# magicat777/Audio-Analyzer-OMEGA

Measured on NVIDIA B200. Metric: stream-seconds of 48 kHz stereo analysed/sec (multi-res FFT+LUFS+TP), higher is better.
Workload: dtype f32 (FFT, combine, K-weighting in a float32 delta-form state, sample peaks of the true-peak meter; its four transforms per frame pair in f16x2; tensor-core GEMM on (hi, lo) half operands with fp32 accumulators for the few-bin resolutions) + f64 (meter statistics)

## Files before the change

audio-analyzer-omega_b200/csrc/omega4_cuda.cu:

```cuda
#include "../../include/omega4_cuda.h"

#include <cuda_runtime.h>
#include <math.h>
#include <stdio.h>
#include <stdlib.h>
#include <string.h>

#include <algorithm>
#include <map>
#include <mutex>
#include <set>
#include <string>
#include <vector>

#include "bars_kernel.cuh"
#include "blockdft_kernel.cuh"
#include "blockdft_tc_kernel.cuh"
#include "fft_core.cuh"
#include "kweight_kernel.cuh"
#include "kweight32_kernel.cuh"
#include "misc_kernels.cuh"
#include "multires_kernel.cuh"
#include "stats_kernel.cuh"
#include "truepeak_kernel.cuh"
#include "truepeak16_kernel.cuh"
#include "waterfall_kernel.cuh"

using namespace o4;

static thread_local std::string g_err;

static int fail(int code, const std::string& msg) {
    g_err = msg;
    return code;
}
#define CK(expr)                                                                                   \
    do {                                                                                           \
        cudaError_t e__ = (expr);                                                                  \
        if (e__ != cudaSuccess) {                                                                  \
            char b__[512];                                                                         \
            snprintf(b__, sizeof b__, "%s failed: %s (%s:%d)", #expr, cudaGetErrorString(e__),     \
                     __FILE__, __LINE__);                                                          \
            return fail(OMEGA4_ERR_CUDA, b__);                                                     \
        }                                                                                          \
    } while (0)

extern "C" const char* omega4_last_error(void) { return g_err.c_str(); }
extern "C" int omega4_abi_version(void) { return OMEGA4_ABI_VERSION; }
extern "C" int omega4_device_count(void) {
    int n = 0;
    if (cudaGetDeviceCount(&n) != cudaSuccess) { cudaGetLastError(); return 0; }
    return n;
}

static int ilog2(int n) { int l = 0; while ((1 << l) < n) ++l; return l; }
static bool is_pow2(int n) { return n > 0 && (n & (n - 1)) == 0; }

struct Twiddles { float2* twM = nullptr; float2* twN = nullptr; float2* tw4W = nullptr; };
static std::mutex g_tw_mu;
static std::map<std::pair<int, int>, Twiddles> g_tw;

static int get_twiddles(int device, int log2m, Twiddles* out) {
    std::lock_guard<std::mutex> lk(g_tw_mu);
    auto key = std::make_pair(device, log2m);
    auto it = g_tw.find(key);
    if (it != g_tw.end()) { *out = it->second; return OMEGA4_OK; }
    const int M = 1 << log2m, N = 2 * M;
    const double two_pi = 6.283185307179586476925287;
    std::vector<float2> a(M), b(M / 2 + 1), c(3 * M + 1);
    for (int e = 0; e < M; ++e) a[e] = make_float2((float)cos(two_pi * e / M), (float)-sin(two_pi * e / M));
    for (int k = 0; k <= M / 2; ++k) b[k] = make_float2((float)cos(two_pi * k / N), (float)-sin(two_pi * k / N));
    for (int j = 0; j <= 3 * M; ++j) c[j] = make_float2((float)cos(two_pi * j / (4.0 * N)), (float)sin(two_pi * j / (4.0 * N)));
    Twiddles t;
    CK(cudaMalloc(&t.twM, a.size() * sizeof(float2)));
    CK(cudaMalloc(&t.twN, b.size() * sizeof(float2)));
    CK(cudaMalloc(&t.tw4W, c.size() * sizeof(float2)));
    CK(cudaMemcpy(t.twM, a.data(), a.size() * sizeof(float2), cudaMemcpyHostToDevice));
    CK(cudaMemcpy(t.twN, b.data(), b.size() * sizeof(float2), cudaMemcpyHostToDevice));
    CK(cudaMemcpy(t.tw4W, c.data(), c.size() * sizeof(float2), cudaMemcpyHostToDevice));
    g_tw[key] = t;
    *out = t;
    return OMEGA4_OK;
}

template <int L>
static int launch_multires_t(const MultiresArgs& a, cudaStream_t s) {
    using S = FftShape<L>;
    const int fpc = a.rounds * S::CONC;
    const long long tiles = (a.n_frames + fpc - 1) / fpc;
    const long long grid = tiles * a.n_ch;
    if (grid <= 0) return OMEGA4_OK;
    if (grid > 2147483647LL) return fail(OMEGA4_ERR_INVALID, "multires grid too large");
    if constexpr (L <= 12) {
        const size_t smem = multires_local_smem_bytes<L>(a.need_cnt, a.n_tb);
        CK(cudaFuncSetAttribute(multires_local_kernel<L>, cudaFuncAttributeMaxDynamicSharedMemorySize, (int)smem));
        multires_local_kernel<L><<<(unsigned)grid, 256, smem, s>>>(a);
    } else {
        const size_t smem = multires_smem_bytes<L>(a.need_cnt);
        CK(cudaFuncSetAttribute(multires_kernel<L>, cudaFuncAttributeMaxDynamicSharedMemorySize, (int)smem));
        multires_kernel<L><<<(unsigned)grid, S::NT, smem, s>>>(a);
    }
    CK(cudaGetLastError());
    return OMEGA4_OK;
}

static int launch_multires(int log2m, const MultiresArgs& a, cudaStream_t s) {
    switch (log2m) {
        case 8: return launch_multires_t<8>(a, s);
        case 9: return launch_multires_t<9>(a, s);
        case 10: return launch_multires_t<10>(a, s);
        case 11: return launch_multires_t<11>(a, s);
        case 12: return launch_multires_t<12>(a, s);
        case 13: return launch_multires_t<13>(a, s);
        case 14: return launch_multires_t<14>(a, s);
    }
    return fail(OMEGA4_ERR_UNSUPPORTED, "fft size must be a power of two in 512 .. 32768");
}

static int default_rounds(int n_frames, int conc) {
    int r = 16;
    while (r > 1 && (long long)r * conc > n_frames) r >>= 1;
    return r;
}

static void fill_truepeak_steps(TruePeakArgs* t) {
    const double two_pi = 6.283185307179586476925287;
    for (int p = 1; p <= 3; ++p) {
        for (int j = 0; j < 16; ++j) {
            const int jj = j < 8 ? j : j - 16;
            t->step[p - 1][j] = make_float2((float)cos(two_pi * p * jj / 64.0), (float)sin(two_pi * p * jj / 64.0));
        }
        t->nyq[p - 1] = (float)cos(two_pi * p / 8.0);
    }
}

static int launch_truepeak(const TruePeakArgs& a, cudaStream_t s) {
    constexpr int L = 11;
    using S = FftShape<L>;
    const size_t smem = truepeak_smem_bytes<L>();
    CK(cudaFuncSetAttribute(truepeak_kernel<L>, cudaFuncAttributeMaxDynamicSharedMemorySize, (int)smem));
    const int ppc = a.rounds * S::CONC;
    const int n_pairs = (a.n_frames + 1) / 2;
    const long long grid = (long long)((n_pairs + ppc - 1) / ppc) * a.n_ch;
    if (grid <= 0) return OMEGA4_OK;
    if (grid > 2147483647LL) return fail(OMEGA4_ERR_INVALID, "truepeak grid too large");
    truepeak_kernel<L><<<(unsigned)grid, S::NT, smem, s>>>(a);
    CK(cudaGetLastError());
    return OMEGA4_OK;
}

static int launch_truepeak16(const TruePeakArgs& a, cudaStream_t s) {
    constexpr int L = 11;
    using S = FftShape<L>;
    const size_t smem = truepeak16_smem_bytes<L>();
    CK(cudaFuncSetAttribute(truepeak16_kernel<L>, cudaFuncAttributeMaxDynamicSharedMemorySize, (int)smem));
    const int ppc = a.rounds * S::CONC;
    const int n_pairs = (a.n_frames + 1) / 2;
    const long long grid = (long long)((n_pairs + ppc - 1) / ppc) * a.n_ch;
    if (grid <= 0) return OMEGA4_OK;
    if (grid > 2147483647LL) return fail(OMEGA4_ERR_INVALID, "truepeak grid too large");
    truepeak16_kernel<L><<<(unsigned)grid, S::NT, smem, s>>>(a);
    CK(cudaGetLastError());
    return OMEGA4_OK;
}

template <bool F64, bool WT>
static int launch_kweight_t(const KweightArgs& a, cudaStream_t s) {
    const size_t smem = kweight_smem_bytes();
    CK(cudaFuncSetAttribute(kweight_kernel<F64, WT>, cudaFuncAttributeMaxDynamicSharedMemorySize, (int)smem));
    const int fpc = a.frames_per_warp * KW_WARPS;
    const long long grid = (long long)((a.n_frames + fpc - 1) / fpc) * a.n_ch;
    if (grid <= 0) return OMEGA4_OK;
    if (grid > 2147483647LL) return fail(OMEGA4_ERR_INVALID, "kweight grid too large");
    kweight_kernel<F64, WT><<<(unsigned)grid, KW_WARPS * 32, smem, s>>>(a);
    CK(cudaGetLastError());
    return OMEGA4_OK;
}

static int launch_kweight(const KweightArgs& a, cudaStream_t s) {
    if (a.x_is_f64) return a.weighted_out ? launch_kweight_t<true, true>(a, s) : launch_kweight_t<true, false>(a, s);
    return a.weighted_out ? launch_kweight_t<false, true>(a, s) : launch_kweight_t<false, false>(a, s);
}

static int launch_kweight32(const Kweight32Args& a, cudaStream_t s) {
    const size_t smem = kweight32_smem_bytes();
    CK(cudaFuncSetAttribute(kweight32_kernel, cudaFuncAttributeMaxDynamicSharedMemorySize, (int)smem));
    const int fpc = a.frames_per_warp * KW32_WARPS;
    const long long grid = (long long)((a.n_frames + fpc - 1) / fpc) * a.n_ch;
    if (grid <= 0) return OMEGA4_OK;
    if (grid > 2147483647LL) return fail(OMEGA4_ERR_INVALID, "kweight grid too large");
    kweight32_kernel<<<(unsigned)grid, KW32_WARPS * 32, smem, s>>>(a);
    CK(cudaGetLastError());
    return OMEGA4_OK;
}

static int launch_stats(const StatsArgs& a, cudaStream_t s) {
    if (a.n_ch <= 0) return OMEGA4_OK;
    if (!a.fresh && a.n_frames == 1 && a.first_frame == 0 && !getenv("OMEGA4_STATS_WALK")) {
        stats_push1_kernel<<<a.n_ch, ST_P1_THREADS, 0, s>>>(a);
    } else if (a.fresh) {
        const size_t smem = stats_smem_bytes<false>();
        CK(cudaFuncSetAttribute(stats_kernel<false>, cudaFuncAttributeMaxDynamicSharedMemorySize, (int)smem));
        stats_kernel<false><<<a.n_ch, ST_THREADS, smem, s>>>(a);
    } else {
        const size_t smem = stats_smem_bytes<true>();
        CK(cudaFuncSetAttribute(stats_kernel<true>, cudaFuncAttributeMaxDynamicSharedMemorySize, (int)smem));
        stats_kernel<true><<<a.n_ch, ST_THREADS, smem, s>>>(a);
    }
    CK(cudaGetLastError());
    return OMEGA4_OK;
}

static int launch_s16_convert(const int16_t* in, long long stream_stride, int il, int n_streams, long long n_frames,
                              float* out, long long out_stride, cudaStream_t s) {
    if (n_streams <= 0 || n_frames <= 0) return OMEGA4_OK;
    if (n_streams > 65535) return fail(OMEGA4_ERR_INVALID, "too many streams for one int16 conversion launch (max 65535)");
    const long long per_stream = n_frames * il;
    dim3 grid((unsigned)((per_stream + 1023) / 1024), (unsigned)n_streams);
    s16_deinterleave_kernel<<<grid, 256, 0, s>>>(in, stream_stride, il, n_frames, out, out_stride);
    CK(cudaGetLastError());
    return OMEGA4_OK;
}

static void mat2_mul(const double* a, const double* b, double* c) {
    double r[4] = {a[0] * b[0] + a[1] * b[2], a[0] * b[1] + a[1] * b[3],
                   a[2] * b[0] + a[3] * b[2], a[2] * b[1] + a[3] * b[3]};
    memcpy(c, r, sizeof r);
}

static void build_biquad(const double* b, const double* a, int order, KwBiquad* q) {
    memset(q, 0, sizeof *q);
    const double a0 = a[0];
    q->b0 = b[0] / a0; q->b1 = b[1] / a0; q->b2 = order >= 2 ? b[2] / a0 : 0.0;
    q->a1 = a[1] / a0; q->a2 = order >= 2 ? a[2] / a0 : 0.0;
    q->pad = 3 * (order + 1);
    if (order >= 2) {
        double zi0, zi1;
        const double m00 = 1.0 + q->a1, m01 = -1.0, m10 = q->a2, m11 = 1.0;
        const double r0 = q->b1 - q->a1 * q->b0, r1 = q->b2 - q->a2 * q->b0;
        const double det = m00 * m11 - m01 * m10;
        zi0 = (r0 * m11 - m01 * r1) / det;
        zi1 = (m00 * r1 - m10 * r0) / det;
        q->yi0 = -zi1 / q->a2;
        q->yi1 = (-zi0 + q->a1 * zi1 / q->a2) / q->a2;
// ... 81 lines not shown
        return OMEGA4_OK;
    }
    void release() { if (p) cudaFree(p); p = nullptr; cap = 0; }
};

struct omega4_bars {
    int device = 0, T = 0, n_valid = 0, p_lo = 0, normalize_max = 0;
    float p_frac = 0.f, scale = 0.8f;
    int* bands = nullptr; float* gain = nullptr; float* sf = nullptr; float* sfc = nullptr;
    DevBuf h_spec, h_out, h_peak, h_state, state_in;
};

static int bars_launch(omega4_bars* b, cudaStream_t s, const float* spec, int n_ch, int n_hops, float* state, int fresh,
                       float* band_values, float* peak_values, DevBuf* state_copy) {
    BarsArgs a;
    memset(&a, 0, sizeof a);
    a.T = b->T; a.n_ch = n_ch; a.n_hops = n_hops; a.n_valid = b->n_valid; a.bands = b->bands; a.gain = b->gain;
    a.sf = b->sf; a.sfc = b->sfc; a.p_lo = b->p_lo; a.p_frac = b->p_frac; a.scale = b->scale;
    a.normalize_max = b->normalize_max; a.fresh = (fresh || !state) ? 1 : 0;
    a.spec = spec; a.bars_out = band_values; a.peaks_out = peak_values; a.state = state;
    const size_t st_bytes = (size_t)n_ch * (1 + b->n_valid) * sizeof(float);
    const size_t smem = bars_smem_bytes(b->T, b->n_valid);
    if (smem > 200 * 1024) return fail(OMEGA4_ERR_UNSUPPORTED, "spectrum too long for the bars kernel");
    if (b->T > 32 * BARS_MAXV) return fail(OMEGA4_ERR_UNSUPPORTED, "spectrum too long for the bars kernel (max 1024 bins)");
    if (b->T <= 512) CK(cudaFuncSetAttribute(bars_kernel<16>, cudaFuncAttributeMaxDynamicSharedMemorySize, (int)smem));
    else CK(cudaFuncSetAttribute(bars_kernel<32>, cudaFuncAttributeMaxDynamicSharedMemorySize, (int)smem));
    a.seg = n_ch >= 1024 ? 4 * BARS_SEG : BARS_SEG;
    const long long grid = (long long)n_ch * ((n_hops + a.seg - 1) / a.seg);
    if (grid > 2147483647LL) return fail(OMEGA4_ERR_INVALID, "bars grid too large");
    if (a.state && !a.fresh && n_hops > a.seg) {
        int rc = state_copy->ensure(st_bytes); if (rc) return rc;
        CK(cudaMemcpyAsync(state_copy->p, a.state, st_bytes, cudaMemcpyDeviceToDevice, s));
        a.state_in = (const float*)state_copy->p;
    }
    if (b->T <= 512) bars_kernel<16><<<(unsigned)grid, BARS_WARPS * 32, smem, s>>>(a);
    else bars_kernel<32><<<(unsigned)grid, BARS_WARPS * 32, smem, s>>>(a);
    CK(cudaGetLastError());
    return OMEGA4_OK;
}

struct BarsReq {
    omega4_bars* b = nullptr;
    float* band_values = nullptr; float* peak_values = nullptr; float* state = nullptr;
    int fresh = 1;
};

struct KernelTime { char name[32]; cudaEvent_t e0, e1; };

struct SideCtx {
    cudaStream_t side = nullptr;
    cudaEvent_t ev_fork = nullptr, ev_tp = nullptr, ev_join = nullptr;
    int ensure() {
        if (side) return OMEGA4_OK;
        CK(cudaStreamCreateWithFlags(&side, cudaStreamNonBlocking));
        CK(cudaEventCreateWithFlags(&ev_fork, cudaEventDisableTiming));
        CK(cudaEventCreateWithFlags(&ev_tp, cudaEventDisableTiming));
        CK(cudaEventCreateWithFlags(&ev_join, cudaEventDisableTiming));
        return OMEGA4_OK;
    }
    void release() {
        if (side) cudaStreamDestroy(side);
        if (ev_fork) cudaEventDestroy(ev_fork);
        if (ev_tp) cudaEventDestroy(ev_tp);
        if (ev_join) cudaEventDestroy(ev_join);
        side = nullptr; ev_fork = ev_tp = ev_join = nullptr;
    }
};

struct omega4_plan {
    int device = 0;
    int sample_rate = 48000, hop = 512, n_res = 0, T = 0, W = OMEGA4_METER_WINDOW;
    double gate = -70.0;
    ResInfo res[OMEGA4_MAX_RES];
    bool disjoint = true;
    int* csr_ptr = nullptr; int* csr_res = nullptr; int* csr_lo = nullptr; float* csr_frac = nullptr;
    double* hann64 = nullptr;
    float* hann32 = nullptr;
    KwBiquad kw_default[2];
    KwBiquad kw[4];
    int kw_nsec = 2, kw_blend = 1, kw_gate = 1;
    double kw_gain = 1.0;
    Twiddles tw_meter;
    float2* tp_rot = nullptr;
    unsigned* tp_rot_h = nullptr;
    SparseSet set_cc;
    SparseSet set_tc;
    bool tensor_default = true;
    DevBuf scratch_lufs, scratch_tp, scratch_mag[OMEGA4_MAX_RES], scratch_q, scratch_f32, scratch_comb, scratch_bstate, scratch_inv;
    DevBuf h_in, h_comb, h_meters, h_state, h_mag[OMEGA4_MAX_RES], h_f64a, h_f64b, h_f64c;
    struct Slot {
        cudaStream_t s = nullptr;
        DevBuf in, in16, comb, met, lufs, tp, state, q, mag[OMEGA4_MAX_RES];
        DevBuf bars, peaks, bstate, bstate_copy;
        SideCtx sc;
    };
#ifndef OMEGA4_HOST_SLOTS
#define OMEGA4_HOST_SLOTS 4
#endif
    static constexpr int N_SLOTS = OMEGA4_HOST_SLOTS;
    Slot slots[N_SLOTS];
    size_t host_chunk_bytes = (size_t)1024 << 20;
    SideCtx sc;
    long long launches = 0;
    std::vector<KernelTime> times;
    size_t n_times = 0;
};

static void set_weighting_k(omega4_plan* p) {
    p->kw[0] = p->kw_default[0]; p->kw[1] = p->kw_default[1];
    p->kw_nsec = 2; p->kw_blend = 1; p->kw_gate = 1; p->kw_gain = 1.0;
}

static double max_pole_radius(const KwBiquad& q) {
    if (q.a2 == 0.0) return fabs(q.a1);
    const double disc = q.a1 * q.a1 - 4.0 * q.a2;
    if (disc < 0.0) return sqrt(q.a2);
    return fmax(fabs(-q.a1 + sqrt(disc)), fabs(-q.a1 - sqrt(disc))) * 0.5;
}

static void to_float(const KwBiquad& s, KwBiquadF* d) {
    d->b0 = (float)s.b0; d->b1 = (float)s.b1; d->b2 = (float)s.b2; d->a1 = (float)s.a1; d->a2 = (float)s.a2;
    d->yi0 = (float)s.yi0; d->yi1 = (float)s.yi1; d->pad = s.pad; d->_align = 0;
    for (int j = 0; j < 5; ++j) for (int e = 0; e < 4; ++e) d->phi[j][e] = (float)s.phi[j][e];
    for (int e = 0; e < 4; ++e) {
        d->cinv_f[e] = (float)s.cinv_f[e]; d->cinv_b[e] = (float)s.cinv_b[e];
        d->c16[e] = (float)s.c16[e]; d->c17[e] = (float)s.c17[e];
    }
    for (int i = 0; i < KW_SUBMAX; ++i) { d->g[i][0] = (float)s.g[i][0]; d->g[i][1] = (float)s.g[i][1]; }
}

static bool is_highpass_biquad(const KwBiquad& q) {
    return q.pad == 9 && q.a2 != 0.0 && fabs(q.b1 + 2.0 * q.b0) <= 1e-12 * fabs(q.b0) && fabs(q.b2 - q.b0) <= 1e-12 * fabs(q.b0);
}

static void build_kw32(const KwBiquad& q, Kw32Sec* o) {
    const double alpha = 1.0 + q.a1 + q.a2, beta = 1.0 - q.a2;
    const double bb = -q.b0 * beta, gamma = alpha / bb;
    o->b0 = (float)q.b0; o->a2 = (float)q.a2; o->gamma = (float)gamma; o->bb = (float)bb;
    const double M[4] = {1.0 - alpha, bb * q.a2, -gamma, q.a2};
    double P[4] = {M[0], M[1], M[2], M[3]};
    for (int i = 0; i < KW_L; ++i) {
        if (i < KW_SUBMAX) { o->g[i][0] = (float)P[0]; o->g[i][1] = (float)P[1]; }
        if (i + 1 == 16) for (int e = 0; e < 4; ++e) o->c16[e] = (float)P[e];
        if (i + 1 == 17) for (int e = 0; e < 4; ++e) o->c17[e] = (float)P[e];
        if (i + 1 < KW_L) mat2_mul(M, P, P);
    }
    for (int k = 0; k < 16; ++k) {
        o->ga0[k] = make_float2(o->g[k + 1][0], o->g[k][0]);
        o->ga1[k] = make_float2(o->g[k + 1][1], o->g[k][1]);
    }
    double Q[4] = {P[0], P[1], P[2], P[3]};
    for (int j = 0; j < 5; ++j) {
        for (int e = 0; e < 4; ++e) o->phi[j][e] = (float)Q[e];
        mat2_mul(Q, Q, Q);
    }
}

static bool use_kweight32(const omega4_plan* p) {
    return p->W == KW_W && p->kw_nsec == 2 && p->kw_blend && p->kw_gain == 1.0 && is_highpass_biquad(p->kw[0]) &&
           is_highpass_biquad(p->kw[1]) && !getenv("OMEGA4_KW_F64");
}

static void fill_weighting(const omega4_plan* p, KweightArgs* k) {
    k->n_sec = p->kw_nsec; k->blend = p->kw_blend; k->rms_gate = p->kw_gate; k->gain = p->kw_gain;
    for (int i = 0; i < p->kw_nsec; ++i) { k->f[i] = p->kw[i]; to_float(p->kw[i], &k->ff[i]); }
    int from = p->kw_nsec;
    while (from > 1 && max_pole_radius(p->kw[from - 1]) < 0.95) --from;
// ... 237 lines not shown
    size_t woff = 0, boff = 0, toff = 0;
    std::vector<std::vector<int>> idx(d->n_res), lo(d->n_res);
    std::vector<std::vector<float>> fr(d->n_res);
    for (int r = 0; r < d->n_res; ++r) {
        ResInfo& ri = p->res[r];
        const int n = d->fft_sizes[r];
        if (!is_pow2(n) || n < 512 || n > 32768) return fail(OMEGA4_ERR_UNSUPPORTED, "fft size must be a power of two in 512 .. 32768");
        ri.n = n; ri.log2m = ilog2(n) - 1; ri.bins = n / 2 + 1; ri.weight = d->res_weight[r];
        if (ri.weight <= 0.f) return fail(OMEGA4_ERR_INVALID, "resolution weight must be positive");
        int rc = upload((void**)&ri.window, d->windows + woff, (size_t)n * sizeof(float));
        if (rc) return rc;
        if (d->bin_weights) { rc = upload((void**)&ri.binw, d->bin_weights + boff, (size_t)ri.bins * sizeof(float)); if (rc) return rc; }
        woff += n; boff += ri.bins;
        const int cnt = d->tb_count[r];
        if (cnt < 0) return fail(OMEGA4_ERR_INVALID, "negative tb_count");
        for (int j = 0; j < cnt; ++j) {
            const int ti = d->tb_idx[toff + j], l = d->tb_lo[toff + j];
            if (ti < 0 || ti >= d->target_bins || l < 0 || l + 1 >= ri.bins)
                return fail(OMEGA4_ERR_INVALID, "combine table entry out of range");
            idx[r].push_back(ti); lo[r].push_back(l); fr[r].push_back(d->tb_frac[toff + j]);
            owners[ti]++;
        }
        toff += cnt;
        rc = get_twiddles(p->device, ri.log2m, &ri.tw);
        if (rc) return rc;
    }
    p->disjoint = true;
    for (int t = 0; t < d->target_bins; ++t) if (owners[t] > 1) p->disjoint = false;
    {
        std::vector<int> ptr(d->target_bins + 1, 0), cres, clo;
        std::vector<float> cfr;
        for (int t = 0; t < d->target_bins; ++t) {
            for (int r = 0; r < d->n_res; ++r)
                for (size_t j = 0; j < idx[r].size(); ++j)
                    if (idx[r][j] == t) { cres.push_back(r); clo.push_back(lo[r][j]); cfr.push_back(fr[r][j]); }
            ptr[t + 1] = (int)cres.size();
        }
        int rc = upload((void**)&p->csr_ptr, ptr.data(), ptr.size() * sizeof(int)); if (rc) return rc;
        rc = upload((void**)&p->csr_res, cres.data(), cres.size() * sizeof(int)); if (rc) return rc;
        rc = upload((void**)&p->csr_lo, clo.data(), clo.size() * sizeof(int)); if (rc) return rc;
        rc = upload((void**)&p->csr_frac, cfr.data(), cfr.size() * sizeof(float)); if (rc) return rc;
    }
    for (int r = 0; r < d->n_res; ++r) {
        ResInfo& ri = p->res[r];
        int mn = 1 << 30, mx = -1;
        for (int l : lo[r]) { if (l < mn) mn = l; if (l > mx) mx = l; }
        if (mx >= 0) { ri.need_lo = mn; ri.need_cnt = mx + 2 - mn; } else { ri.need_lo = 0; ri.need_cnt = 0; }
        if (r == 0)
            for (int t = 0; t < d->target_bins; ++t)
                if (owners[t] == 0) { idx[0].push_back(t); lo[0].push_back(-1); fr[0].push_back(0.f); }
        ri.n_tb = (int)idx[r].size();
        int rc = upload((void**)&ri.tb_idx, idx[r].data(), idx[r].size() * sizeof(int)); if (rc) return rc;
        rc = upload((void**)&ri.tb_lo, lo[r].data(), lo[r].size() * sizeof(int)); if (rc) return rc;
        rc = upload((void**)&ri.tb_frac, fr[r].data(), fr[r].size() * sizeof(float)); if (rc) return rc;
    }
    if (p->disjoint) {
        int rc = build_sparse_set(p, d, idx, lo, false, &p->set_cc); if (rc) return rc;
        rc = build_sparse_set(p, d, idx, lo, true, &p->set_tc); if (rc) return rc;
    }
    int rc = upload((void**)&p->hann64, d->meter_hann, (size_t)p->W * sizeof(double)); if (rc) return rc;
    std::vector<float> h32(p->W);
    for (int i = 0; i < p->W; ++i) h32[i] = (float)d->meter_hann[i];
    rc = upload((void**)&p->hann32, h32.data(), h32.size() * sizeof(float)); if (rc) return rc;
    build_biquad(d->kw_coeffs + 0, d->kw_coeffs + 3, 2, &p->kw_default[0]);
    build_biquad(d->kw_coeffs + 6, d->kw_coeffs + 9, 2, &p->kw_default[1]);
    set_weighting_k(p);
    rc = get_twiddles(p->device, ilog2(p->W), &p->tw_meter); if (rc) return rc;
    {
        const int W = p->W;
        std::vector<float2> rot((size_t)3 * W);
        const double two_pi = 6.283185307179586476925287;
        for (int ph = 1; ph <= 3; ++ph)
            for (int k = 0; k < W; ++k) {
                float2 v;
                if (k == W / 2) v = make_float2((float)cos(two_pi * ph / 8.0), 0.f);
                else {
                    const double f = (k < W / 2) ? (double)k : (double)k - W;
                    const double ang = two_pi * f * ph / (4.0 * W);
                    v = make_float2((float)cos(ang), (float)sin(ang));
                }
                rot[(size_t)(ph - 1) * W + k] = v;
            }
        rc = upload((void**)&p->tp_rot, rot.data(), rot.size() * sizeof(float2)); if (rc) return rc;
        std::vector<unsigned> roth(rot.size());
        for (size_t i = 0; i < rot.size(); ++i) {
            const __half2 h = __floats2half2_rn(rot[i].x, rot[i].y);
            memcpy(&roth[i], &h, sizeof(unsigned));
        }
        rc = upload((void**)&p->tp_rot_h, roth.data(), roth.size() * sizeof(unsigned)); if (rc) return rc;
    }
    return OMEGA4_OK;
}

extern "C" omega4_plan* omega4_plan_create(const omega4_plan_desc* desc, int device) {
    if (!desc) { fail(OMEGA4_ERR_INVALID, "desc is NULL"); return nullptr; }
    int ndev = 0;
    if (cudaGetDeviceCount(&ndev) != cudaSuccess || ndev == 0) {
        cudaGetLastError();
        fail(OMEGA4_ERR_NO_DEVICE, "no CUDA device visible: libomega4_cuda has no CPU fallback");
        return nullptr;
    }
    if (device < 0 || device >= ndev) { fail(OMEGA4_ERR_INVALID, "bad device index"); return nullptr; }
    if (cudaSetDevice(device) != cudaSuccess) { fail(OMEGA4_ERR_CUDA, "cudaSetDevice failed"); return nullptr; }
    omega4_plan* p = new omega4_plan();
    p->device = device;
    if (const char* e = getenv("OMEGA4_TENSOR")) p->tensor_default = atoi(e) != 0;
    if (const char* e = getenv("OMEGA4_HOST_CHUNK_MB")) {
        long mb = atol(e);
        if (mb >= 16 && mb <= 16384) p->host_chunk_bytes = (size_t)mb << 20;
    }
    if (plan_build(p, desc) != OMEGA4_OK) { std::string keep = g_err; omega4_plan_destroy(p); g_err = keep; return nullptr; }
    return p;
}

static void stream_ctx_release(omega4_plan* p);

extern "C" void omega4_plan_destroy(omega4_plan* p) {
    if (!p) return;
    cudaSetDevice(p->device);
    stream_ctx_release(p);
    for (int r = 0; r < OMEGA4_MAX_RES; ++r) {
        ResInfo& ri = p->res[r];
        cudaFree(ri.window); cudaFree(ri.binw); cudaFree(ri.tb_idx); cudaFree(ri.tb_lo); cudaFree(ri.tb_frac);
        p->scratch_mag[r].release(); p->h_mag[r].release();
    }
    cudaFree(p->csr_ptr); cudaFree(p->csr_res); cudaFree(p->csr_lo); cudaFree(p->csr_frac);
    cudaFree(p->hann64); cudaFree(p->hann32); cudaFree(p->tp_rot); cudaFree(p->tp_rot_h);
    p->scratch_lufs.release(); p->scratch_tp.release(); p->scratch_q.release(); p->scratch_f32.release(); p->scratch_inv.release();
    p->scratch_comb.release(); p->scratch_bstate.release();
    p->set_cc.release(); p->set_tc.release();
    p->h_in.release(); p->h_comb.release(); p->h_meters.release(); p->h_state.release();
    p->h_f64a.release(); p->h_f64b.release(); p->h_f64c.release();
    for (auto& sl : p->slots) {
        sl.in.release(); sl.comb.release(); sl.met.release(); sl.lufs.release(); sl.tp.release(); sl.state.release();
        sl.q.release(); sl.in16.release(); sl.sc.release();
        sl.bars.release(); sl.peaks.release(); sl.bstate.release(); sl.bstate_copy.release();
        for (auto& m : sl.mag) m.release();
        if (sl.s) cudaStreamDestroy(sl.s);
    }
    for (auto& t : p->times) { cudaEventDestroy(t.e0); cudaEventDestroy(t.e1); }
    p->sc.release();
    cudaGetLastError();
    delete p;
}

extern "C" long long omega4_plan_launches(const omega4_plan* p) { return p ? p->launches : 0; }

extern "C" int omega4_plan_set_weighting(omega4_plan* p, const omega4_weighting* w) {
    if (!p) return fail(OMEGA4_ERR_INVALID, "plan is NULL");
    if (!w) { set_weighting_k(p); return OMEGA4_OK; }
    if (w->n_sections < 0 || w->n_sections > 4) return fail(OMEGA4_ERR_INVALID, "0..4 weighting sections");
    if (w->blend && w->n_sections != 2) return fail(OMEGA4_ERR_INVALID, "the K blend needs exactly two sections");
    KwBiquad tmp[4];
    for (int i = 0; i < w->n_sections; ++i) {
        const int order = w->order[i];
        if (order != 1 && order != 2) return fail(OMEGA4_ERR_UNSUPPORTED, "weighting sections must be first or second order");
        if (w->a[i][0] == 0.0 || w->a[i][1] == 0.0 || (order == 2 && w->a[i][2] == 0.0))
            return fail(OMEGA4_ERR_UNSUPPORTED, "weighting sections need non-zero denominator coefficients");
        build_biquad(w->b[i], w->a[i], order, &tmp[i]);
    }
    for (int i = 0; i < w->n_sections; ++i) p->kw[i] = tmp[i];
    p->kw_nsec = w->n_sections; p->kw_blend = w->blend ? 1 : 0; p->kw_gate = w->rms_gate ? 1 : 0;
    p->kw_gain = w->blend ? 1.0 : w->gain;
    return OMEGA4_OK;
}

struct Bracket {
    omega4_plan* p; cudaStream_t s; bool on; KernelTime* kt = nullptr;
    Bracket(omega4_plan* p_, cudaStream_t s_, bool on_, const char* name) : p(p_), s(s_), on(on_) {
        p->launches++;
        if (!on) return;
        if (p->n_times == p->times.size()) {
            KernelTime t; memset(&t, 0, sizeof t);
            cudaEventCreate(&t.e0); cudaEventCreate(&t.e1);
            p->times.push_back(t);
        }
        kt = &p->times[p->n_times++];
        snprintf(kt->name, sizeof kt->name, "%s", name);
        cudaEventRecord(kt->e0, s);
    }
    ~Bracket() { if (on && kt) cudaEventRecord(kt->e1, s); }
};

extern "C" int omega4_plan_kernel_times(omega4_plan* p, char* names, float* ms, int max_n) {
    if (!p) return fail(OMEGA4_ERR_INVALID, "plan is NULL");
    int n = 0;
    for (size_t i = 0; i < p->n_times && n < max_n; ++i, ++n) {
        float t = 0.f;
        if (cudaEventElapsedTime(&t, p->times[i].e0, p->times[i].e1) != cudaSuccess) { cudaGetLastError(); t = -1.f; }
        if (names) { memcpy(names + 32 * n, p->times[i].name, 32); }
        if (ms) ms[n] = t;
    }
    return n;
}

template <int BN>
static int launch_blockdft_gemm_t(const BlockDftGemmArgs& a, cudaStream_t s) {
    const size_t smem = blockdft_gemm_smem_bytes<BN>();
    CK(cudaFuncSetAttribute(blockdft_gemm_kernel<BN>, cudaFuncAttributeMaxDynamicSharedMemorySize, (int)smem));
    const long long grid = (long long)((a.nb + BD_BM - 1) / BD_BM) * a.n_ch;
    if (grid > 2147483647LL) return fail(OMEGA4_ERR_INVALID, "blockdft grid too large");
    blockdft_gemm_kernel<BN><<<(unsigned)grid, BD_THREADS, smem, s>>>(a);
    CK(cudaGetLastError());
    return OMEGA4_OK;
}

static int launch_blockdft_gemm(int bn, const BlockDftGemmArgs& a, cudaStream_t s) {
    if (a.nb <= 0 || a.n_ch <= 0) return OMEGA4_OK;
    switch (bn) {
        case 32: return launch_blockdft_gemm_t<32>(a, s);
// ... 10 lines not shown
    if (timing) p->n_times = 0;
    if (((uintptr_t)x & 15) != 0 || (ch_stride % 4) != 0)
        return fail(OMEGA4_ERR_INVALID, "samples must be 16-byte aligned with ch_stride a multiple of 4");
    const bool want_meters = meters || lufs || tp;
    const bool concurrent = want_meters && (flags & OMEGA4_FLAG_CONCURRENT_METERS);
    const bool stats_aside = !concurrent && meters && combined && !(flags & OMEGA4_FLAG_SERIAL_STATS);
    cudaStream_t ms = s;
    cudaStream_t ss = s;
    if (concurrent || stats_aside) {
        int rc = sc->ensure(); if (rc) return rc;
        ss = sc->side;
    }
    if (concurrent) {
        ms = sc->side;
        CK(cudaEventRecord(sc->ev_fork, s));
        CK(cudaStreamWaitEvent(ms, sc->ev_fork, 0));
    }
    const bool fused = p->disjoint;
    int first[OMEGA4_MAX_RES];
    bool use_sparse[OMEGA4_MAX_RES] = {false};
    bool any_sparse = false;
    const bool tensor = p->set_tc.n > 0 && (p->tensor_default ? !(flags & OMEGA4_FLAG_NO_TENSOR) : (flags & OMEGA4_FLAG_TENSOR) != 0);
    const SparseSet& set = tensor ? p->set_tc : p->set_cc;
    for (int r = 0; r < p->n_res; ++r) {
        use_sparse[r] = combined && fused && set.of_res[r] >= 0 && !(mags && mags[r]) &&
                        !(flags & OMEGA4_FLAG_NO_BLOCKDFT);
        any_sparse = any_sparse || use_sparse[r];
        long long need = (long long)p->res[r].n - hist;
        first[r] = need <= 0 ? 0 : (int)((need + p->hop - 1) / p->hop - 1);
    }
    int sp_j0 = 1 << 30;
    for (int r = 0; r < p->n_res; ++r)
        if (use_sparse[r]) { const int j = first[r] + 1 - set.sp[set.of_res[r]].B; if (j < sp_j0) sp_j0 = j; }
    const int sp_nb = any_sparse ? n_hops - sp_j0 : 0;
    float* row_inv = nullptr;
    int inv_from_kw = -1;
#if TC_F16
    if (tensor && any_sparse && sp_nb > 0) {
        int rc = p->scratch_inv.ensure((size_t)n_ch * sp_nb * sizeof(float)); if (rc) return rc;
        row_inv = (float*)p->scratch_inv.p;
    }
#endif
    if (want_meters) {
        const size_t nser = (size_t)n_ch * n_hops * sizeof(double);
        if (!lufs) { int rc = p->scratch_lufs.ensure(nser); if (rc) return rc; lufs = (double*)p->scratch_lufs.p; }
        if (!tp) { int rc = p->scratch_tp.ensure(nser); if (rc) return rc; tp = (double*)p->scratch_tp.p; }
        long long need = (long long)p->W - hist;
        const int first_m = need <= 0 ? 0 : (int)((need + p->hop - 1) / p->hop - 1);
        if (use_kweight32(p)) {
            Kweight32Args k;
            memset(&k, 0, sizeof k);
            k.x = x; k.ch_stride = ch_stride; k.frame_stride = p->hop;
            k.frame_off0 = (long long)p->hop - p->W;
            k.n_ch = n_ch; k.n_frames = n_hops; k.first_frame = first_m;
            k.frames_per_warp = n_hops >= 64 ? 8 : (n_hops >= 8 ? 2 : 1);
            k.hann = p->hann32; k.lufs_out = lufs; k.rms_gate = p->kw_gate;
            if (row_inv && !concurrent && p->hop * 4 == p->W && first_m < n_hops && !getenv("OMEGA4_NO_SCALE_FOLD")) {
                k.hop_inv = row_inv; k.hop_inv_nb = sp_nb; k.hop_inv_j0 = sp_j0;
                inv_from_kw = first_m;
            }
            build_kw32(p->kw[0], &k.s[0]); build_kw32(p->kw[1], &k.s[1]);
            Bracket b(p, ms, timing, "kweight_lufs");
            int rc = launch_kweight32(k, ms);
            if (rc) return rc;
        } else {
            KweightArgs k;
            memset(&k, 0, sizeof k);
            k.x = x; k.x_is_f64 = 0; k.ch_stride = ch_stride; k.frame_stride = p->hop;
            k.frame_off0 = (long long)p->hop - p->W;
            k.n_ch = n_ch; k.n_frames = n_hops; k.first_frame = first_m;
            k.frames_per_warp = n_hops >= 64 ? 8 : (n_hops >= 8 ? 2 : 1);
            k.hann = p->hann64; k.lufs_out = lufs; k.weighted_out = nullptr;
            fill_weighting(p, &k);
            Bracket b(p, ms, timing, "kweight_lufs");
            int rc = launch_kweight(k, ms);
            if (rc) return rc;
        }
        {
            TruePeakArgs t;
            memset(&t, 0, sizeof t);
            t.x = x; t.x_is_f64 = 0; t.ch_stride = ch_stride; t.frame_stride = p->hop;
            t.frame_off0 = (long long)p->hop - p->W;
            t.n_ch = n_ch; t.n_frames = n_hops; t.first_frame = first_m;
            t.rounds = default_rounds((n_hops + 1) / 2, 2);
            t.window = p->hann32; t.twM = p->tw_meter.twM; t.rot = p->tp_rot; t.rot_h = p->tp_rot_h;
            fill_truepeak_steps(&t);
            t.tp_out = tp;
            Bracket b(p, s, timing, "true_peak");
            const bool exact_tp = (flags & OMEGA4_FLAG_EXACT_TRUE_PEAK) || getenv("OMEGA4_TP_F32");
            int rc = exact_tp ? launch_truepeak(t, s) : launch_truepeak16(t, s);
            if (rc) return rc;
        }
        if (meters) {
            if (concurrent || stats_aside) {
                CK(cudaEventRecord(sc->ev_tp, s));
                CK(cudaStreamWaitEvent(ss, sc->ev_tp, 0));
            }
            StatsArgs st;
            memset(&st, 0, sizeof st);
            st.lufs = lufs; st.tp = tp; st.n_ch = n_ch; st.n_frames = n_hops; st.first_frame = first_m;
            st.gate = p->gate; st.out = meters;
            st.fresh = (state == nullptr) || (flags & OMEGA4_FLAG_FRESH_METERS) ? 1 : 0;
            if (!state) {
                int rc = p->h_state.ensure((size_t)n_ch * ST_STATE * sizeof(double));
                if (rc) return rc;
                state = (double*)p->h_state.p;
            }
            st.state = state;
            Bracket b(p, ss, timing, "meter_stats");
            int rc = launch_stats(st, ss);
            if (rc) return rc;
        }
        if (concurrent || stats_aside) CK(cudaEventRecord(sc->ev_join, ss));
    }
    float* mag_ptr[OMEGA4_MAX_RES];
    for (int r = 0; r < p->n_res; ++r) {
        ResInfo& ri = p->res[r];
        mag_ptr[r] = mags ? mags[r] : nullptr;
        if (combined && !fused && !mag_ptr[r]) {
            int rc = p->scratch_mag[r].ensure((size_t)n_ch * n_hops * ri.bins * sizeof(float));
            if (rc) return rc;
            mag_ptr[r] = (float*)p->scratch_mag[r].p;
        }
        if (!combined && !mag_ptr[r]) continue;
        if (use_sparse[r]) continue;
        MultiresArgs a;
        memset(&a, 0, sizeof a);
        a.x = x; a.ch_stride = ch_stride; a.frame_stride = p->hop; a.frame_off0 = (long long)p->hop - ri.n;
        a.n_ch = n_ch; a.n_frames = n_hops; a.first_frame = first[r];
        a.rounds = default_rounds(n_hops, (1 << ri.log2m) >= 4096 ? 1 : 4096 >> ri.log2m);
        a.window = ri.window; a.binw = ri.binw; a.twM = ri.tw.twM; a.twN = ri.tw.twN;
        a.mag_out = mag_ptr[r]; a.cplx_out = nullptr;
        a.comb_out = (combined && fused) ? combined : nullptr;
        a.T = p->T; a.n_tb = ri.n_tb; a.tb_idx = ri.tb_idx; a.tb_lo = ri.tb_lo; a.tb_frac = ri.tb_frac;
        a.wnum = ri.weight; a.wden = ri.weight;
        a.need_lo = ri.need_lo; a.need_cnt = (combined && fused) ? ri.need_cnt : 0;
        char name[32];
        snprintf(name, sizeof name, "multires_fft_%d", ri.n);
        Bracket b(p, s, timing, name);
        int rc = launch_multires(ri.log2m, a, s);
        if (rc) return rc;
    }
    if (any_sparse) {
        const int j0 = sp_j0, nb = sp_nb;
        const float* Q = nullptr;
        const bool fusedx = tensor && set.fusable;
        if (nb > 0) {
            const size_t qbytes = fusedx ? (size_t)n_ch * set.nkx * n_hops * sizeof(float2)
                                         : (size_t)n_ch * nb * set.qs * sizeof(float);
            int rc = qbuf->ensure(qbytes);
            if (rc) return rc;
            Q = (float*)qbuf->p;
            if (tensor) {
                BlockDftTcArgs g;
                memset(&g, 0, sizeof g);
                g.x = x; g.ch_stride = ch_stride; g.hop = p->hop; g.n_ch = n_ch; g.j0 = j0; g.nb = nb;
                g.n_halves = set.n_halves; g.Eimg = set.Eimg; g.Q = (float*)qbuf->p; g.qs = set.qs;
#if TC_F16
                {
                    HopScaleArgs h;
                    h.x = x; h.ch_stride = ch_stride; h.hop = p->hop; h.n_ch = n_ch; h.j0 = j0; h.nb = nb;
                    h.ncols = inv_from_kw >= 0 ? inv_from_kw - j0 : nb;
                    h.inv = row_inv;
                    g.row_inv = h.inv; g.e_inv = set.e_inv;
                    const long long rows = (long long)n_ch * h.ncols;
                    if (rows > 0) {
                        Bracket b(p, s, timing, "blockdft_row_scale");
                        hopblock_scale_kernel<<<(unsigned)((rows + 7) / 8), 256, 0, s>>>(h);
                        CK(cudaGetLastError());
                    }
                }
#endif
                if (fusedx) {
// ... 924 lines not shown
```

audio-analyzer-omega_b200/csrc/truepeak_kernel.cuh:

```cuda
#pragma once
#include "fft_core.cuh"

namespace o4 {

struct TruePeakArgs {
    const void* x;
    int x_is_f64;
    long long ch_stride;
    long long frame_stride;
    long long frame_off0;
    int n_ch;
    int n_frames;
    int first_frame;
    int rounds;
    const float* window;
    const float2* twM;
    const float2* rot;
    const unsigned* rot_h;
    double* tp_out;
    float2 step[3][16];
    float nyq[3];
};

template <int LOG2M>
__global__ void __launch_bounds__(256, 2)
truepeak_kernel(const __grid_constant__ TruePeakArgs a) {
    using S = FftShape<LOG2M>;
    constexpr int M = S::M, TPF = S::TPF, CONC = S::CONC, BUF = S::BUF;
    constexpr int WARPS = TPF / 32;
    static_assert(TPF >= 32 && S::NT == 256 && LOG2M <= 12, "true-peak kernel: whole warps per transform, local FFT variant");
    extern __shared__ __align__(16) unsigned char smem_raw[];
    float2* bufs = reinterpret_cast<float2*>(smem_raw);
    float2* red_all = bufs + (size_t)CONC * (BUF + M);

    const int tid = threadIdx.x;
    const int g = tid / TPF;
    const int t = tid % TPF;
    float2* X = bufs + (size_t)g * (BUF + M);
    float2* Z = X + BUF;
    float2* red = red_all + g * 2 * WARPS;

    const int pairs_per_cta = a.rounds * CONC;
    const int n_pairs = (a.n_frames + 1) >> 1;
    const int tiles_per_ch = (n_pairs + pairs_per_cta - 1) / pairs_per_cta;
    const int ch = blockIdx.x / tiles_per_ch;
    const int tile = blockIdx.x % tiles_per_ch;

    LocalTwFull<LOG2M> st;
    {
        LocalTw<LOG2M> st4;
        load_local_twiddles<LOG2M>(st4, a.twM, t);
        expand_local_twiddles<LOG2M>(st4, st);
    }
    const float inv_m = 1.0f / (float)M;
    auto nop = []() {};
    auto group_max2 = [&](float2 v, int slot) -> float2 {
#pragma unroll
        for (int o = 16; o > 0; o >>= 1) {
            v.x = fmaxf(v.x, __shfl_xor_sync(0xffffffffu, v.x, o));
            v.y = fmaxf(v.y, __shfl_xor_sync(0xffffffffu, v.y, o));
        }
        if ((t & 31) == 0) red[slot * WARPS + (t >> 5)] = v;
        group_sync<TPF>(g);
        float2 m = red[slot * WARPS];
#pragma unroll
        for (int w = 1; w < WARPS; ++w) { const float2 o = red[slot * WARPS + w]; m.x = fmaxf(m.x, o.x); m.y = fmaxf(m.y, o.y); }
        return m;
    };

    const int zt = zaddr<LOG2M>(t);
    const float2 rbase1 = __ldg(a.rot + t), rbase2 = __ldg(a.rot + M + t), rbase3 = __ldg(a.rot + 2 * M + t);
    auto load_pair = [&](int pi, float2 (&v)[16]) {
        const int fa = 2 * pi, fb = fa + 1;
        const bool act_a = (fa < a.n_frames) && (fa >= a.first_frame);
        const bool act_b = (fb < a.n_frames) && (fb >= a.first_frame);
#pragma unroll
        for (int j = 0; j < 16; ++j) v[j] = make_float2(0.f, 0.f);
        if (!(act_a || act_b)) return;
        const long long off_a = (long long)ch * a.ch_stride + a.frame_off0 + (long long)fa * a.frame_stride + t;
        if (a.x_is_f64) {
            const double* pa = reinterpret_cast<const double*>(a.x) + off_a;
            const double* pb = pa + a.frame_stride;
#pragma unroll
            for (int j = 0; j < 16; ++j) {
                if (act_a) v[j].x = (float)pa[j * TPF];
                if (act_b) v[j].y = (float)pb[j * TPF];
            }
        } else {
            const float* pa = reinterpret_cast<const float*>(a.x) + off_a;
            const float* pb = pa + a.frame_stride;
#pragma unroll
            for (int j = 0; j < 16; ++j) {
                if (act_a) v[j].x = __ldg(pa + j * TPF);
                if (act_b) v[j].y = __ldg(pb + j * TPF);
            }
        }
    };
    float2 v[16];
    load_pair(tile * pairs_per_cta + g, v);
    for (int r = 0; r < a.rounds; ++r) {
        const int pi = tile * pairs_per_cta + r * CONC + g;
// ... 62 lines not shown
```

Baseline: 284,200.

## Replace f16x2 true-peak FFT kernel with tensor-core mma-based FFT

Result: slower. 273,200, median of 6 (-3.9%).

```diff
diff --git a/audio-analyzer-omega_b200/csrc/omega4_cuda.cu b/audio-analyzer-omega_b200/csrc/omega4_cuda.cu
--- a/audio-analyzer-omega_b200/csrc/omega4_cuda.cu
+++ b/audio-analyzer-omega_b200/csrc/omega4_cuda.cu
@@ -23,7 +23,7 @@
 #include "multires_kernel.cuh"
 #include "stats_kernel.cuh"
 #include "truepeak_kernel.cuh"
-#include "truepeak16_kernel.cuh"
+#include "truepeak_mma_kernel.cuh"
 #include "waterfall_kernel.cuh"
 
 using namespace o4;
@@ -149,17 +149,12 @@
     return OMEGA4_OK;
 }
 
-static int launch_truepeak16(const TruePeakArgs& a, cudaStream_t s) {
-    constexpr int L = 11;
-    using S = FftShape<L>;
-    const size_t smem = truepeak16_smem_bytes<L>();
-    CK(cudaFuncSetAttribute(truepeak16_kernel<L>, cudaFuncAttributeMaxDynamicSharedMemorySize, (int)smem));
-    const int ppc = a.rounds * S::CONC;
+static int launch_truepeak_mma(const TruePeakArgs& a, cudaStream_t s) {
     const int n_pairs = (a.n_frames + 1) / 2;
-    const long long grid = (long long)((n_pairs + ppc - 1) / ppc) * a.n_ch;
+    const long long grid = (long long)((n_pairs + a.rounds - 1) / a.rounds) * a.n_ch;
     if (grid <= 0) return OMEGA4_OK;
     if (grid > 2147483647LL) return fail(OMEGA4_ERR_INVALID, "truepeak grid too large");
-    truepeak16_kernel<L><<<(unsigned)grid, S::NT, smem, s>>>(a);
+    truepeak_mma_kernel<<<(unsigned)grid, TPM_THREADS, 0, s>>>(a);
     CK(cudaGetLastError());
     return OMEGA4_OK;
 }
@@ -407,7 +402,7 @@
     double kw_gain = 1.0;
     Twiddles tw_meter;
     float2* tp_rot = nullptr;
-    unsigned* tp_rot_h = nullptr;
+    float2* tp_mma_tab = nullptr;
     SparseSet set_cc;
     SparseSet set_tc;
     bool tensor_default = true;
@@ -811,12 +806,9 @@
                 rot[(size_t)(ph - 1) * W + k] = v;
             }
         rc = upload((void**)&p->tp_rot, rot.data(), rot.size() * sizeof(float2)); if (rc) return rc;
-        std::vector<unsigned> roth(rot.size());
-        for (size_t i = 0; i < rot.size(); ++i) {
-            const __half2 h = __floats2half2_rn(rot[i].x, rot[i].y);
-            memcpy(&roth[i], &h, sizeof(unsigned));
-        }
-        rc = upload((void**)&p->tp_rot_h, roth.data(), roth.size() * sizeof(unsigned)); if (rc) return rc;
+        std::vector<float2> tab(TPM_TAB);
+        truepeak_mma_tables(tab.data());
+        rc = upload((void**)&p->tp_mma_tab, tab.data(), tab.size() * sizeof(float2)); if (rc) return rc;
     }
     return OMEGA4_OK;
 }
@@ -854,7 +846,7 @@
         p->scratch_mag[r].release(); p->h_mag[r].release();
     }
     cudaFree(p->csr_ptr); cudaFree(p->csr_res); cudaFree(p->csr_lo); cudaFree(p->csr_frac);
-    cudaFree(p->hann64); cudaFree(p->hann32); cudaFree(p->tp_rot); cudaFree(p->tp_rot_h);
+    cudaFree(p->hann64); cudaFree(p->hann32); cudaFree(p->tp_rot); cudaFree(p->tp_mma_tab);
     p->scratch_lufs.release(); p->scratch_tp.release(); p->scratch_q.release(); p->scratch_f32.release(); p->scratch_inv.release();
     p->scratch_comb.release(); p->scratch_bstate.release();
     p->set_cc.release(); p->set_tc.release();
@@ -1031,13 +1023,13 @@
             t.x = x; t.x_is_f64 = 0; t.ch_stride = ch_stride; t.frame_stride = p->hop;
             t.frame_off0 = (long long)p->hop - p->W;
             t.n_ch = n_ch; t.n_frames = n_hops; t.first_frame = first_m;
-            t.rounds = default_rounds((n_hops + 1) / 2, 2);
-            t.window = p->hann32; t.twM = p->tw_meter.twM; t.rot = p->tp_rot; t.rot_h = p->tp_rot_h;
+            t.window = p->hann32; t.twM = p->tw_meter.twM; t.rot = p->tp_rot; t.tpm_tab = p->tp_mma_tab;
             fill_truepeak_steps(&t);
             t.tp_out = tp;
             Bracket b(p, s, timing, "true_peak");
             const bool exact_tp = (flags & OMEGA4_FLAG_EXACT_TRUE_PEAK) || getenv("OMEGA4_TP_F32");
-            int rc = exact_tp ? launch_truepeak(t, s) : launch_truepeak16(t, s);
+            t.rounds = exact_tp ? default_rounds((n_hops + 1) / 2, 2) : default_rounds((n_hops + 1) / 2, 1);
+            int rc = exact_tp ? launch_truepeak(t, s) : launch_truepeak_mma(t, s);
             if (rc) return rc;
         }
         if (meters) {
diff --git a/audio-analyzer-omega_b200/csrc/truepeak_kernel.cuh b/audio-analyzer-omega_b200/csrc/truepeak_kernel.cuh
--- a/audio-analyzer-omega_b200/csrc/truepeak_kernel.cuh
+++ b/audio-analyzer-omega_b200/csrc/truepeak_kernel.cuh
@@ -16,7 +16,7 @@
     const float* window;
     const float2* twM;
     const float2* rot;
-    const unsigned* rot_h;
+    const float2* tpm_tab;
     double* tp_out;
     float2 step[3][16];
     float nyq[3];
diff --git a/audio-analyzer-omega_b200/csrc/truepeak_mma_kernel.cuh b/audio-analyzer-omega_b200/csrc/truepeak_mma_kernel.cuh
--- /dev/null
+++ b/audio-analyzer-omega_b200/csrc/truepeak_mma_kernel.cuh
@@ -0,0 +1,278 @@
+#pragma once
+#include <cuda_fp16.h>
+#include <math.h>
+#include "truepeak_kernel.cuh"
+
+namespace o4 {
+
+constexpr int TPM_THREADS = 128;
+constexpr int TPM_W256 = 4 * 32 * 64;
+constexpr int TPM_MATS = TPM_W256 + 256;
+constexpr int TPM_TAB = TPM_MATS + 4 * 256 / 2;
+
+inline void truepeak_mma_tables(float2* tab) {
+    const double two_pi = 6.283185307179586476925287;
+    auto w = [&](long long num, long long den) {
+        const double ang = -two_pi * (double)(num % den) / (double)den;
+        return make_float2((float)cos(ang), (float)sin(ang));
+    };
+    for (int p = 0; p < 4; ++p)
+        for (int k2 = 0; k2 < 32; ++k2)
+            for (int m = 0; m < 64; m += 2) {
+                const float2 w0 = w((long long)k2 * (4 * m + p), 8192), w1 = w((long long)k2 * (4 * (m + 1) + p), 8192);
+                tab[(p * 32 + k2) * 64 + m] = make_float2(w0.x, w1.x);
+                tab[(p * 32 + k2) * 64 + m + 1] = make_float2(w0.y, w1.y);
+            }
+    for (int x = 0; x < 256; ++x) tab[TPM_W256 + x] = w(x, 256);
+    auto f8 = [&](int r, int c) {
+        const double ang = two_pi * (double)(((r & 7) * (c & 7)) & 7) / 8.0;
+        if ((r < 8) == (c < 8)) return cos(ang);
+        return r < 8 ? sin(ang) : -sin(ang);
+    };
+    float* mats = reinterpret_cast<float*>(tab + TPM_MATS);
+    for (int p = 0; p < 4; ++p)
+        for (int r = 0; r < 16; ++r)
+            for (int c = 0; c < 16; ++c) {
+                double v = f8(r, c);
+                if (p > 0) {
+                    const int j = c & 7;
+                    const double ang = two_pi * p * (j < 4 ? j : j - 8) / 32.0, br = cos(ang), bi = sin(ang);
+                    v = c < 8 ? f8(r, j) * br - f8(r, 8 + j) * bi : -f8(r, j) * bi - f8(r, 8 + j) * br;
+                }
+                mats[p * 256 + r * 16 + c] = (float)v;
+            }
+}
+
+__device__ __forceinline__ unsigned h2u(__half2 h) { return *reinterpret_cast<unsigned*>(&h); }
+__device__ __forceinline__ unsigned pack_h2(float lo, float hi) { return h2u(__floats2half2_rn(lo, hi)); }
+__device__ __forceinline__ float2 u2f2(unsigned u) { return __half22float2(*reinterpret_cast<__half2*>(&u)); }
+
+__device__ __forceinline__ void mma16816(float (&d)[4], const unsigned (&a)[4], unsigned b0, unsigned b1) {
+    asm volatile("mma.sync.aligned.m16n8k16.row.col.f32.f16.f16.f32 {%0,%1,%2,%3}, {%4,%5,%6,%7}, {%8,%9}, "
+                 "{%10,%11,%12,%13};\n"
+                 : "=f"(d[0]), "=f"(d[1]), "=f"(d[2]), "=f"(d[3])
+                 : "r"(a[0]), "r"(a[1]), "r"(a[2]), "r"(a[3]), "r"(b0), "r"(b1),
+                   "f"(0.f), "f"(0.f), "f"(0.f), "f"(0.f));
+}
+__device__ __forceinline__ unsigned movmatrix_t(unsigned x) {
+    unsigned y;
+    asm volatile("movmatrix.sync.aligned.m8n8.trans.b16 %0, %1;\n" : "=r"(y) : "r"(x));
+    return y;
+}
+__device__ __forceinline__ void ldmatrix_x4_t(unsigned (&r)[4], unsigned saddr) {
+    asm volatile("ldmatrix.sync.aligned.m8n8.x4.trans.shared.b16 {%0,%1,%2,%3}, [%4];\n"
+                 : "=r"(r[0]), "=r"(r[1]), "=r"(r[2]), "=r"(r[3]) : "r"(saddr) : "memory");
+}
+
+__device__ __forceinline__ void tw_frag(float (&c)[4], float2 wr, float2 wi) {
+    const float2 re = make_float2(c[0], c[1]), im = make_float2(c[2], c[3]);
+    const float2 t = __fmul2_rn(im, wi), u = __fmul2_rn(im, wr);
+    const float2 r = __ffma2_rn(re, wr, make_float2(-t.x, -t.y)), i = __ffma2_rn(re, wi, u);
+    c[0] = r.x; c[1] = r.y; c[2] = i.x; c[3] = i.y;
+}
+__device__ __forceinline__ float2 f2re(float2 a, float2 b) { return make_float2(a.x, b.x); }
+__device__ __forceinline__ float2 f2im(float2 a, float2 b) { return make_float2(a.y, b.y); }
+
+__device__ __forceinline__ unsigned tpm_off(int block, int row, int swz) { return (unsigned)((block * 8 + (row ^ swz)) * 16); }
+
+__global__ void __launch_bounds__(TPM_THREADS, 3)
+truepeak_mma_kernel(const __grid_constant__ TruePeakArgs a) {
+    constexpr int M = 2048;
+    __shared__ __align__(128) unsigned char xbuf[4][8192];
+    __shared__ float2 red[2][4];
+
+    const int tid = threadIdx.x, w = tid >> 5, lane = tid & 31, g = lane >> 2, t = lane & 3;
+    const int n_pairs = (a.n_frames + 1) >> 1;
+    const int tiles_per_ch = (n_pairs + a.rounds - 1) / a.rounds;
+    const int ch = blockIdx.x / tiles_per_ch;
+    const int tile = blockIdx.x % tiles_per_ch;
+
+    const float2* w256 = a.tpm_tab + TPM_W256;
+    const float* mats = reinterpret_cast<const float*>(a.tpm_tab + TPM_MATS);
+    unsigned am[4][4];
+#pragma unroll
+    for (int p = 0; p < 4; ++p) {
+        const float* m = mats + p * 256;
+        am[p][0] = pack_h2(__ldg(m + g * 16 + 2 * t), __ldg(m + g * 16 + 2 * t + 1));
+        am[p][1] = pack_h2(__ldg(m + (g + 8) * 16 + 2 * t), __ldg(m + (g + 8) * 16 + 2 * t + 1));
+        am[p][2] = pack_h2(__ldg(m + g * 16 + 2 * t + 8), __ldg(m + g * 16 + 2 * t + 9));
+        am[p][3] = pack_h2(__ldg(m + (g + 8) * 16 + 2 * t + 8), __ldg(m + (g + 8) * 16 + 2 * t + 9));
+    }
+    float2 tw64r[4], tw64i[4];
+#pragma unroll
+    for (int p = 0; p < 4; ++p) {
+        const float2 w0 = __ldg(w256 + (((2 * t) * (4 * g + p)) & 255)), w1 = __ldg(w256 + (((2 * t + 1) * (4 * g + p)) & 255));
+        tw64r[p] = f2re(w0, w1); tw64i[p] = f2im(w0, w1);
+    }
+    float2 tw32i[3];
+#pragma unroll
+    for (int k = 1; k < 4; ++k) tw32i[k - 1] = __ldg(w256 + ((8 * g * k) & 255));
+
+    const unsigned sbase = (unsigned)__cvta_generic_to_shared(&xbuf[0][0]);
+    const float4* tw4 = reinterpret_cast<const float4*>(a.tpm_tab);
+    const float inv_m = 1.0f / (float)M;
+
+    for (int r = 0; r < a.rounds; ++r) {
+        const int pi = tile * a.rounds + r;
+        const int fa = 2 * pi, fb = fa + 1;
+        const bool act_a = (fa < a.n_frames) && (fa >= a.first_frame);
+        const bool act_b = (fb < a.n_frames) && (fb >= a.first_frame);
+        if (!(act_a || act_b)) continue;
+
+        float2 v[2][2][4];
+        {
+            const float* pa = reinterpret_cast<const float*>(a.x) + (long long)ch * a.ch_stride + a.frame_off0 + (long long)fa * a.frame_stride;
+            const float* pb = pa + a.frame_stride;
+#pragma unroll
+            for (int th = 0; th < 2; ++th)
+#pragma unroll
+                for (int e = 0; e < 2; ++e)
+#pragma unroll
+                    for (int h = 0; h < 4; ++h) {
+                        const int n = g + 8 * th + 16 * w + 64 * (2 * t + e) + 512 * h;
+                        float xa = act_a ? __ldg(pa + n) : 0.f, xb = act_b ? __ldg(pb + n) : 0.f;
+                        v[th][e][h] = make_float2(xa, xb);
+                        if (a.window) { const float wv = __ldg(a.window + n); v[th][e][h] = __fmul2_rn(v[th][e][h], make_float2(wv, wv)); }
+                    }
+        }
+        float2 pk = make_float2(0.f, 0.f);
+#pragma unroll
+        for (int th = 0; th < 2; ++th)
+#pragma unroll
+            for (int e = 0; e < 2; ++e)
+#pragma unroll
+                for (int h = 0; h < 4; ++h) { pk.x = fmaxf(pk.x, fabsf(v[th][e][h].x)); pk.y = fmaxf(pk.y, fabsf(v[th][e][h].y)); }
+#pragma unroll
+        for (int o = 16; o > 0; o >>= 1) {
+            pk.x = fmaxf(pk.x, __shfl_xor_sync(0xffffffffu, pk.x, o));
+            pk.y = fmaxf(pk.y, __shfl_xor_sync(0xffffffffu, pk.y, o));
+        }
+        if (lane == 0) red[0][w] = pk;
+        __syncthreads();
+#pragma unroll
+        for (int i = 0; i < 4; ++i) { pk.x = fmaxf(pk.x, red[0][i].x); pk.y = fmaxf(pk.y, red[0][i].y); }
+        const float sa = pk.x > 1e-20f ? 1.f / pk.x : 0.f, sb = pk.y > 1e-20f ? 1.f / pk.y : 0.f;
+
+#pragma unroll
+        for (int th = 0; th < 2; ++th) {
+            unsigned bre[4], bim[4];
+            float2 xo[2][4];
+#pragma unroll
+            for (int e = 0; e < 2; ++e) {
+                const float2 sab = make_float2(sa, sb);
+                float2 x0 = __fmul2_rn(v[th][e][0], sab), x1 = __fmul2_rn(v[th][e][1], sab);
+                float2 x2 = __fmul2_rn(v[th][e][2], sab), x3 = __fmul2_rn(v[th][e][3], sab);
+                bf4(x0, x1, x2, x3);
+                xo[e][0] = x0;
+                xo[e][1] = cmul(x1, __ldg(w256 + ((8 * (2 * t + e)) & 255)));
+                xo[e][2] = cmul(x2, __ldg(w256 + ((16 * (2 * t + e)) & 255)));
+                xo[e][3] = cmul(x3, __ldg(w256 + ((24 * (2 * t + e)) & 255)));
+            }
+#pragma unroll
+            for (int k = 0; k < 4; ++k) { bre[k] = pack_h2(xo[0][k].x, xo[1][k].x); bim[k] = pack_h2(xo[0][k].y, xo[1][k].y); }
+#pragma unroll
+            for (int k = 0; k < 4; ++k) {
+                float c[4];
+                mma16816(c, am[0], bre[k], bim[k]);
+                const int k2 = k + 4 * g, n1 = 2 * t + 8 * th + 16 * w;
+                const float4 tw = __ldg(tw4 + ((0 * 32 + k2) * 64 + n1) / 2);
+                tw_frag(c, make_float2(tw.x, tw.y), make_float2(tw.z, tw.w));
+                const unsigned o = tpm_off(k2 * 2, th + 2 * w, g) + 4 * t;
+                asm volatile("st.shared.u32 [%0], %1;\n" ::"r"(sbase + o), "r"(pack_h2(c[0], c[1])) : "memory");
+                asm volatile("st.shared.u32 [%0], %1;\n" ::"r"(sbase + o + 128), "r"(pack_h2(c[2], c[3])) : "memory");
+            }
+        }
+        __syncthreads();
+
+        float2 zn = make_float2(0.f, 0.f);
+#pragma unroll 1
+        for (int tau = 0; tau < 8; tau += 2) {
+            unsigned ld[4];
+            {
+                const int mat = lane >> 3, k2 = tau + (mat >> 1) + 8 * w;
+                ldmatrix_x4_t(ld, sbase + tpm_off(k2 * 2 + (mat & 1), lane & 7, (k2 >> 2) & 7));
+            }
+#pragma unroll
+            for (int s = 0; s < 2; ++s) {
+                const int k2 = tau + s + 8 * w;
+                float c[4];
+                mma16816(c, am[0], ld[2 * s], ld[2 * s + 1]);
+                tw_frag(c, tw64r[0], tw64i[0]);
+                mma16816(c, am[0], pack_h2(c[0], c[1]), pack_h2(c[2], c[3]));
+                const unsigned zre = movmatrix_t(pack_h2(c[0], c[1])), zim = movmatrix_t(pack_h2(c[2], c[3]));
+                if (k2 == 0) {
+                    const float zr = u2f2(__shfl_sync(0xffffffffu, zre, 2)).x, zi = u2f2(__shfl_sync(0xffffffffu, zim, 2)).x;
+                    zn = make_float2(zr, zi);
+                }
+#pragma unroll
+                for (int p = 1; p <= 3; ++p) {
+                    float d[4];
+                    mma16816(d, am[p], zre, zim);
+                    if (k2 == 0 && t == 0) {
+                        const float sn = (p == 2) ? 1.f : 0.70710678118654752f, sg = (g & 1) ? sn : -sn;
+                        d[0] = fmaf(sg, zn.y, d[0]);
+                        d[2] = fmaf(sg, zn.x, d[2]);
+                    }
+                    tw_frag(d, tw64r[p], tw64i[p]);
+                    mma16816(d, am[0], pack_h2(d[0], d[1]), pack_h2(d[2], d[3]));
+                    const float4 tw = __ldg(tw4 + ((p * 32 + k2) * 64 + 2 * t + 8 * g) / 2);
+                    tw_frag(d, make_float2(tw.x, tw.y), make_float2(tw.z, tw.w));
+                    const unsigned o = (unsigned)p * 8192u + tpm_off(((g * 4 + (k2 & 3)) * 2), k2 >> 2, g) + 4 * t;
+                    asm volatile("st.shared.u32 [%0], %1;\n" ::"r"(sbase + o), "r"(pack_h2(d[0], d[1])) : "memory");
+                    asm volatile("st.shared.u32 [%0], %1;\n" ::"r"(sbase + o + 128), "r"(pack_h2(d[2], d[3])) : "memory");
+                }
+            }
+        }
+        __syncthreads();
+
+        float mre = 0.f, mim = 0.f;
+#pragma unroll 1
+        for (int p = 1; p <= 3; ++p) {
+#pragma unroll
+            for (int th = 0; th < 2; ++th) {
+                const int m1h = th + 2 * w;
+                float c[4][4];
+#pragma unroll
+                for (int kk = 0; kk < 4; kk += 2) {
+                    unsigned ld[4];
+                    const int mat = lane >> 3;
+                    ldmatrix_x4_t(ld, sbase + (unsigned)p * 8192u + tpm_off((m1h * 4 + kk + (mat >> 1)) * 2 + (mat & 1), lane & 7, m1h));
+                    mma16816(c[kk], am[0], ld[0], ld[1]);
+                    mma16816(c[kk + 1], am[0], ld[2], ld[3]);
+                }
+#pragma unroll
+                for (int k = 1; k < 4; ++k) tw_frag(c[k], make_float2(tw32i[k - 1].x, tw32i[k - 1].x), make_float2(tw32i[k - 1].y, tw32i[k - 1].y));
+#pragma unroll
+                for (int e = 0; e < 2; ++e) {
+                    float2 x0 = make_float2(c[0][e], c[0][e + 2]), x1 = make_float2(c[1][e], c[1][e + 2]);
+                    float2 x2 = make_float2(c[2][e], c[2][e + 2]), x3 = make_float2(c[3][e], c[3][e + 2]);
+                    bf4(x0, x1, x2, x3);
+                    mre = fmaxf(fmaxf(fmaxf(mre, fabsf(x0.x)), fmaxf(fabsf(x1.x), fabsf(x2.x))), fabsf(x3.x));
+                    mim = fmaxf(fmaxf(fmaxf(mim, fabsf(x0.y)), fmaxf(fabsf(x1.y), fabsf(x2.y))), fabsf(x3.y));
+                }
+            }
+        }
+#pragma unroll
+        for (int o = 16; o > 0; o >>= 1) {
+            mre = fmaxf(mre, __shfl_xor_sync(0xffffffffu, mre, o));
+            mim = fmaxf(mim, __shfl_xor_sync(0xffffffffu, mim, o));
+        }
+        if (lane == 0) red[1][w] = make_float2(mre, mim);
+        __syncthreads();
+        if (tid == 0) {
+            float2 po = red[1][0];
+#pragma unroll
+            for (int i = 1; i < 4; ++i) { po.x = fmaxf(po.x, red[1][i].x); po.y = fmaxf(po.y, red[1][i].y); }
+            if (act_a) {
+                const double peak = (double)pk.x * (double)fmaxf(1.f, po.x * inv_m);
+                a.tp_out[(size_t)ch * a.n_frames + fa] = (peak < 1e-10) ? -100.0 : 20.0 * log10(peak);
+            }
+            if (act_b) {
+                const double peak = (double)pk.y * (double)fmaxf(1.f, po.y * inv_m);
+                a.tp_out[(size_t)ch * a.n_frames + fb] = (peak < 1e-10) ? -100.0 : 20.0 * log10(peak);
+            }
+        }
+    }
+}
+
+}
```
